# software-mansion/smelter

Measured on NVIDIA H100. Metric: 4K composited frames/sec (16-input grid) per GPU, higher is better.
Workload: dtype f32 math on u8 planes (f16 resampler scratch)

## Files before the change

smelter_b200/csrc/resample_tma3.cuh:

```cuda
#pragma once

namespace tma_int {
using namespace tma;

constexpr int kGroups = 3;

template <int S>
struct Cfg {
    static constexpr int P = 8;
    static constexpr int OUT = P / S;
    static constexpr int TAPS = 6 * S + 1;
    static constexpr int A = kLead<S>;
    static constexpr int NST = (A + S * (OUT - 1) + TAPS + P - 1) / P;
    static __host__ __device__ constexpr int last_stage(int j) { return (A + S * j + TAPS - 1) / P; }
    static __host__ __device__ constexpr int nout() {
        int m = 1 << 30;
        for (int j = 0; j < OUT; j++) {
            int c = OUT * (32 - last_stage(j)) + j;
            m = c < m ? c : m;
        }
        return m;
    }
    static constexpr int NOUT = nout();
    static constexpr int RROWS = S == 4 ? 54 : 28;
    static constexpr int RROW_BYTES = 32 * 3 * OUT * 4;
    static constexpr int RING_BYTES = RROWS * RROW_BYTES;
    static constexpr int GROUP_BYTES = kStageBytes + RING_BYTES;
    static constexpr int SMEM = kGroups * GROUP_BYTES + kTailBytes;
};

template <int S, int SRC>
__global__ void __launch_bounds__(32 * kWarps * kGroups, 1) k_resample_tma3(const FusedJob *jobs, const FusedPiece *pieces, const int *piece_begin,
                                                                            int n_virtual_blocks) {
    using K = Cfg<S>;
    using It = ChunkIter<S, 1>;
    constexpr int P = K::P, OUT = K::OUT, TAPS = K::TAPS, A = K::A, NST = K::NST;
    constexpr bool NV12 = SRC == 1;
    extern __shared__ __align__(128) unsigned char smem_all[];
    const int lane = threadIdx.x, warp = threadIdx.y % kWarps, grp = threadIdx.y / kWarps, tid = warp * 32 + lane;
    unsigned char *tail = smem_all + kGroups * K::GROUP_BYTES;
    const float *s_thr = reinterpret_cast<const float *>(tail + kThrOff);
    unsigned char *smem = smem_all + (size_t)grp * K::GROUP_BYTES;
    const uint32_t stage0 = smem_u32(smem);
    float *ring = reinterpret_cast<float *>(smem + kStageBytes);
    const uint32_t bar0 = smem_u32(tail + kBarOff) + 16u * (uint32_t)grp;
    const uint32_t kaddr = setup_block<kGroups>(tail, [] {});
    const int vb = blockIdx.x * kGroups + grp;
    if (vb >= n_virtual_blocks) return;

    Stash<It> *stash = stash_slots<It, kGroups>(tail, grp);
    uint32_t step = 0;
    It it;
    it.init(jobs, pieces, __ldg(piece_begin + vb), __ldg(piece_begin + vb + 1));

    Chunk cur = it.next();
    if (!cur.valid) return;
    if (tid == 0) issue<NV12, 1>(jobs, cur, stage0, bar0);
    uint32_t nchunk = 0;

    while (cur.valid) {
        Stash<It> *const parked = stash + (step & 1u);
        {
            const Chunk nxt = it.next();
            if (tid == 0) { parked->it = it; parked->nxt = nxt; }
        }
        const bool cur_tma = cur.nrows > 0;
        const FusedJob &J = jobs[cur.job];
        const int W = J.src.width, H = J.src.height, chei = H >> 1;
        const bool full_range = J.src.full_range != 0;
        const float nk16 = full_range ? 0.0f : -K16, rcp_y = full_range ? 1.0f : RCP_Y, rcp_c = full_range ? 1.0f : RCP_C;
        const uint32_t sb = stage0;
        if (cur_tma) {
            mbar_wait(bar0, nchunk & 1u);
            replicate_edges<NV12>(smem, cur.x0, cur.nrows, W, tid, grp);
            const LaneWords<NV12> lw(cur.x0, lane);
            for (int r = cur.r0 + warp; r < cur.r0 + cur.nrows; r += kWarps) {
                uint32_t yw[2], v[6];
                fetch_row<NV12>(sb, lw, r, cur.r0, chei, yw, v);
                float2 prg[P];
                float pb[P];
                convert_run(yw, v, nk16, rcp_y, rcp_c, kaddr, prg, pb);
                float2 arg[OUT];
                float ab[OUT];
#pragma unroll
                for (int j = 0; j < OUT; j++) { arg[j] = make_float2(0.f, 0.f); ab[j] = 0.f; }
#pragma unroll
                for (int s = 0; s < NST; s++) {
#pragma unroll
                    for (int i = 0; i < P; i++) {
#pragma unroll
                        for (int j = 0; j < OUT; j++) {
                            const int t = P * s + i - A - S * j;
                            if (t >= 0 && t < TAPS) arg[j] = fma2(prg[i], splat(c_wint[S][t]), arg[j]);
                        }
#pragma unroll
                        for (int j = 0; j < OUT; j += 2) {
                            const int t0 = P * s + i - A - S * j, t1 = t0 - S;
                            const bool a0 = t0 >= 0 && t0 < TAPS, a1 = t1 >= 0 && t1 < TAPS;
                            if (a0 && a1) {
                                const float2 d = fma2(splat(pb[i]), c_wpair[S][a0 ? t0 : 0], make_float2(ab[j], ab[j + 1]));
                                ab[j] = d.x; ab[j + 1] = d.y;
                            } else if (a0) {
                                ab[j] = fmaf(pb[i], c_wint[S][a0 ? t0 : 0], ab[j]);
                            } else if (a1) {
                                ab[j + 1] = fmaf(pb[i], c_wint[S][a1 ? t1 : 0], ab[j + 1]);
                            }
                        }
                    }
                    if (s + 1 < NST) {
#pragma unroll
                        for (int j = 0; j < OUT; j++)
                            if (K::last_stage(j) > s) {
                                arg[j].x = __shfl_up_sync(0xffffffffu, arg[j].x, 1);
                                arg[j].y = __shfl_up_sync(0xffffffffu, arg[j].y, 1);
                                ab[j] = __shfl_up_sync(0xffffffffu, ab[j], 1);
                            }
                    }
                }
                {
                    const float inv = c_winv[S];
                    float *dst = ring + (size_t)(r % K::RROWS) * (K::RROW_BYTES / 4) + lane * 3 * OUT;
#pragma unroll
                    for (int j = 0; j < OUT; j += 2) {
                        const float2 fr = __half22float2(__floats2half2_rn(arg[j].x * inv, arg[j + 1].x * inv));
                        const float2 fg = __half22float2(__floats2half2_rn(arg[j].y * inv, arg[j + 1].y * inv));
                        const float2 fb = __half22float2(__floats2half2_rn(ab[j] * inv, ab[j + 1] * inv));
                        *reinterpret_cast<float2 *>(dst + j) = fr;
                        *reinterpret_cast<float2 *>(dst + OUT + j) = fg;
                        *reinterpret_cast<float2 *>(dst + 2 * OUT + j) = fb;
                    }
                }
            }
            nchunk++;
        }
        group_sync(grp);
        if (tid == 0) issue<NV12, 1>(jobs, parked->nxt, stage0, bar0);
        if (cur.last) {
            const int tv = J.taps_v;
            const float *lbase = ring + lane * 3 * OUT;
            constexpr int ROWF = K::RROW_BYTES / 4;
            const int row_end = min(cur.o0 + kWarps, cur.oy_end);
            auto col_of = [&](int j) { return OUT * (lane - K::last_stage(j)) + j; };
            auto owned = [&](int oa, bool (&own)[OUT / 2]) {
                const int ncols = min(K::NOUT, J.dst_w - cur.ox0);
#pragma unroll
                for (int j = 0; j < OUT; j += 2) {
                    const int col = col_of(j);
                    own[j / 2] = false;
                    if (J.direct_map == nullptr || col < 0 || col >= ncols || oa >= row_end) continue;
                    const int X = J.fx + cur.ox0 + col, Y = J.fy + oa;
                    own[j / 2] = (int)__ldg(J.direct_map + (Y / kDirectTileH) * J.map_w + X / kDirectTileW) == J.direct_id;
                }
            };
            auto emit = [&](const uint32_t (&pa)[OUT], const uint32_t (&pb)[OUT], int oa, const bool (&own)[OUT / 2]) {
#pragma unroll
                for (int j = 0; j < OUT; j += 2) {
                    if (!own[j / 2]) continue;
                    emit_yuv_2x2(J, J.fx + cur.ox0 + col_of(j), J.fy + oa, pa[j], pa[j + 1], pb[j], pb[j + 1]);
                }
            };
            auto one_row = [&](int oy, uint32_t (&px)[OUT]) {
                const int fv = __ldg(J.first_v + oy);
                const float *wv = J.w_v + (size_t)oy * tv;
                float2 acc[3 * OUT / 2];
#pragma unroll
                for (int k = 0; k < 3 * OUT / 2; k++) acc[k] = make_float2(0.f, 0.f);
                for (int t = 0; t < tv; t++) {
                    const float wt = __ldg(wv + t);
                    const int row = min(max(fv + t, 0), H - 1);
                    const float *p = lbase + (row % K::RROWS) * ROWF;
#pragma unroll
                    for (int k = 0; k < 3 * OUT / 2; k++) acc[k] = fma2(*reinterpret_cast<const float2 *>(p + 2 * k), splat(wt), acc[k]);
                }
                encode_store<OUT>(J, acc, oy, s_thr, cur.ox0, K::NOUT, col_of, px);
            };
            if (J.v_same) {
                if (warp < kWarps / 2) {
                    const int oa = cur.o0 + 2 * warp, ob = oa + 1;
                    const int fa = __ldg(J.first_v) + S * oa;
                    bool own[OUT / 2];
                    owned(oa, own);
                    if (ob < row_end && fa >= 0 && fa + S + TAPS - 1 <= H - 1) {
                        float2 aa[3 * OUT / 2], bb2[3 * OUT / 2];
#pragma unroll
                        for (int k = 0; k < 3 * OUT / 2; k++) { aa[k] = make_float2(0.f, 0.f); bb2[k] = make_float2(0.f, 0.f); }
                        const int slot0 = fa % K::RROWS, nwrap = K::RROWS - slot0;
                        const float *p0 = lbase + slot0 * ROWF;
#pragma unroll
                        for (int u = 0; u < TAPS + S; u++) {
                            const float *p = p0 + (u >= nwrap ? (u - K::RROWS) * ROWF : u * ROWF);
                            float2 v[3 * OUT / 2];
#pragma unroll
                            for (int k = 0; k < 3 * OUT / 2; k++) v[k] = *reinterpret_cast<const float2 *>(p + 2 * k);
                            if (u < TAPS) {
#pragma unroll
                                for (int k = 0; k < 3 * OUT / 2; k++) aa[k] = fma2(v[k], splat(c_wint[S][u < TAPS ? u : 0]), aa[k]);
                            }
                            if (u >= S) {
#pragma unroll
                                for (int k = 0; k < 3 * OUT / 2; k++) bb2[k] = fma2(v[k], splat(c_wint[S][u >= S ? u - S : 0]), bb2[k]);
                            }
                        }
                        uint32_t pa[OUT], pb[OUT];
                        encode_store<OUT>(J, aa, oa, s_thr, cur.ox0, K::NOUT, col_of, pa);
                        encode_store<OUT>(J, bb2, ob, s_thr, cur.ox0, K::NOUT, col_of, pb);
                        emit(pa, pb, oa, own);
                    } else {
                        uint32_t pa[OUT], pb[OUT];
                        if (oa < row_end) one_row(oa, pa);
                        if (ob < row_end) { one_row(ob, pb); emit(pa, pb, oa, own); }
                    }
                }
            } else {
                const int oy = cur.o0 + warp;
                uint32_t pz[OUT];
                if (oy < row_end) one_row(oy, pz);
            }
            group_sync(grp);
        }
        cur = parked->nxt; it = parked->it; step++;
    }
}

}
```

smelter_b200/csrc/kernels.cu:

```cuda
#include <cuda_fp16.h>
#include <cuda_runtime.h>

#include <cstdio>
#include <cstdlib>
#include <atomic>
#include <cstring>

#include "kernels.h"

namespace smr {
namespace dev {

#include "ptx_helpers.cuh"

__device__ float c_u8n[256];
__device__ float c_dec[256];
__device__ float c_thr[256];
#define ENC_KEY0 ((127 - 13) << 5)
#define ENC_KEYS ((13 << 5) + 1)
__device__ unsigned char c_enc0[420];
__device__ float c_yl[256];
#define ENC1_KEY0 ((127 - 13) << 8)
#define ENC1_KEYS ((13 << 8) + 1)
__device__ unsigned char c_enc1[ENC1_KEYS + 3];
// ... 342 lines not shown
__device__ __forceinline__ float4 rs_load(const Tables &T, const Tex &s, int x, int y) {
    if (s.kind == TEX_F16) {
        const uint2 raw = __ldg(reinterpret_cast<const uint2 *>(s.p0 + (size_t)y * s.pitch0) + x);
        __half2 a = *reinterpret_cast<const __half2 *>(&raw.x), b = *reinterpret_cast<const __half2 *>(&raw.y);
        float2 fa = __half22float2(a), fb = __half22float2(b);
        return make_float4(fa.x, fa.y, fb.x, fb.y);
    }
    uchar4 p = node_texel(T, s, x, y);
    return make_float4(T.dec[p.x], T.dec[p.y], T.dec[p.z], T.u8n[p.w]);
}

__device__ __forceinline__ void rs_store(const Tables &T, const ResampleJob &J, int x, int y, float4 r) {
    if (J.dst_f16) {
        __half2 a = __floats2half2_rn(r.x, r.y), b = __floats2half2_rn(r.z, r.w);
        uint2 raw;
        raw.x = *reinterpret_cast<unsigned int *>(&a);
        raw.y = *reinterpret_cast<unsigned int *>(&b);
        reinterpret_cast<uint2 *>(J.dst + (size_t)y * J.dst_pitch)[x] = raw;
    } else {
        uchar4 o = make_uchar4((unsigned char)srgb_encode(T, r.x), (unsigned char)srgb_encode(T, r.y),
                               (unsigned char)srgb_encode(T, r.z), (unsigned char)unorm8(r.w));
        reinterpret_cast<uchar4 *>(J.dst + (size_t)y * J.dst_pitch)[x] = o;
    }
}

__global__ void __launch_bounds__(256) k_resample(const ResampleJob *jobs) {
    __shared__ Tables T;
    load_tables(T);
    const ResampleJob &J = jobs[blockIdx.z];
    int px = blockIdx.x * blockDim.x + threadIdx.x, py = blockIdx.y * blockDim.y + threadIdx.y;
    if (px >= J.dst_w || py >= J.dst_h) return;
    const Tex &S = J.src;
    if (J.box_fx * J.box_fy > 1) {
        float4 sum = make_float4(0.f, 0.f, 0.f, 0.f);
        for (int dy = 0; dy < J.box_fy; dy++)
            for (int dx = 0; dx < J.box_fx; dx++) {
                int sx = min(px * J.box_fx + dx, S.width - 1), sy = min(py * J.box_fy + dy, S.height - 1);
                float4 t = rs_load(T, S, sx, sy);
                sum.x += t.x; sum.y += t.y; sum.z += t.z; sum.w += t.w;
            }
        float d = (float)((unsigned)J.box_fx * (unsigned)J.box_fy);
        rs_store(T, J, px, py, make_float4(sum.x / d, sum.y / d, sum.z / d, sum.w / d));
        return;
    }
    int o = J.axis == 1 ? py : px;
    int max_src = (J.axis == 1 ? S.height : S.width) - 1;
    int max_perp = (J.axis == 1 ? S.width : S.height) - 1;
    int perp = min(max((J.axis == 1 ? px : py) + J.perp_offset, 0), max_perp);
    const float *w = J.weights + (size_t)o * J.taps;
    int first = __ldg(J.first + o);
    float4 sum = make_float4(0.f, 0.f, 0.f, 0.f);
    for (int t = 0; t < J.taps; t++) {
        float wt = __ldg(w + t);
        if (wt == 0.0f) continue;
        int src = min(max(first + t, 0), max_src);
        float4 tx = J.axis == 1 ? rs_load(T, S, perp, src) : rs_load(T, S, src, perp);
        sum.x = fmaf(tx.x, wt, sum.x);
        sum.y = fmaf(tx.y, wt, sum.y);
        sum.z = fmaf(tx.z, wt, sum.z);
        sum.w = fmaf(tx.w, wt, sum.w);
    }
    float inv = __ldg(J.inv_wsum + o);
    rs_store(T, J, px, py, make_float4(sum.x * inv, sum.y * inv, sum.z * inv, sum.w * inv));
}

int launch_resample(const ResampleJob *jobs_dev, const ResampleJob *jobs_host, int n, Stream s) {
    if (n <= 0) return 0;
    int mw = 1, mh = 1;
    for (int i = 0; i < n; i++) {
        mw = jobs_host[i].dst_w > mw ? jobs_host[i].dst_w : mw;
        mh = jobs_host[i].dst_h > mh ? jobs_host[i].dst_h : mh;
    }
    dim3 b(32, 8), g((mw + 31) / 32, (mh + 7) / 8, n);
    k_resample<<<g, b, 0, (cudaStream_t)s>>>(jobs_dev);
    return check_launch("k_resample") ? 1 : -1;
}

#define W64_TW 64
#define W64_WARPS 8
#define W64_RING 64

__constant__ float c_wint[5][32];
__constant__ float c_winv[5];
__constant__ float2 c_wpair[5][32];

void set_int_weights(int S, const float *weights_dev, const float *inv_dev, int taps, Stream s) {
    cudaMemcpyToSymbolAsync(c_wint, weights_dev, sizeof(float) * taps, sizeof(float) * 32 * S, cudaMemcpyDeviceToDevice, (cudaStream_t)s);
    cudaMemcpyToSymbolAsync(c_winv, inv_dev, sizeof(float), sizeof(float) * S, cudaMemcpyDeviceToDevice, (cudaStream_t)s);
    float *pair = nullptr;
    cudaGetSymbolAddress((void **)&pair, c_wpair);
    pair += 2 * 32 * S;
    cudaMemsetAsync(pair, 0, sizeof(float2) * 32, (cudaStream_t)s);
    cudaMemcpy2DAsync(pair, sizeof(float2), weights_dev, sizeof(float), sizeof(float), taps, cudaMemcpyDeviceToDevice, (cudaStream_t)s);
    if (taps > S)
        cudaMemcpy2DAsync(pair + 2 * S + 1, sizeof(float2), weights_dev, sizeof(float), sizeof(float), taps - S,
                          cudaMemcpyDeviceToDevice, (cudaStream_t)s);
}

template <int S>
struct W64 {
    static constexpr int SS = S == 0 ? 4 : S;
    static constexpr int TAPS = 6 * SS + 1;
    static constexpr int SPAN = (W64_TW - 1) * SS + TAPS + 3;
    static constexpr int ROWLEN = S == 0 ? ((SPAN + 2 + 7) & ~7) : (((SPAN + SPAN / (2 * SS) + 2) + 7) & ~7);
    struct Smem {
        Tables T;
        __half2 ring[W64_RING][3][W64_TW / 2];
        float4 srow[W64_WARPS][ROWLEN];
        float hw[S == 0 ? TAPS * W64_TW : 1];
    };
    static __device__ __forceinline__ int pos(int i) { return S == 0 ? i : i + i / (2 * SS); }
};

__device__ __forceinline__ void prefetch_l2_span(const uint8_t *p, int bytes, const uint8_t *lo, const uint8_t *hi) {
    unsigned long long a = (unsigned long long)(p < lo ? lo : p), e = (unsigned long long)(p + bytes < hi ? p + bytes : hi);
    a = (a + 15ull) & ~15ull;
    if (e <= a + 16ull) return;
    const unsigned size = (unsigned)((e - a) & ~15ull);
    asm volatile("cp.async.bulk.prefetch.L2.global [%0], %1;" ::"l"(a), "r"(size) : "memory");
}

template <int S, int SRC>
__global__ void __launch_bounds__(32 * W64_WARPS, 3) k_resample_fused_int(const FusedJob *jobs, const FusedPiece *pieces,
                                                                            const int *piece_begin) {
    constexpr bool NV12 = SRC == 1, IL = SRC >= 2;
    using K = W64<S>;
    constexpr int TAPS = K::TAPS;
    constexpr int WIN = S + TAPS;
    extern __shared__ __align__(16) unsigned char fs_raw[];
    typename K::Smem &M = *reinterpret_cast<typename K::Smem *>(fs_raw);
    load_tables(M.T);
    const int lane = threadIdx.x, warp = threadIdx.y;
    for (int pi = __ldg(piece_begin + blockIdx.x); pi < __ldg(piece_begin + blockIdx.x + 1); pi++) {
    const FusedPiece P = pieces[pi];
    const FusedJob &J = jobs[P.job];
    const int th = S == 0 ? J.taps_h : TAPS;
    const int ox0 = P.strip * W64_TW;
    const int oy_begin = P.oy_begin, oy_end = P.oy_end;
    const Tex &src = J.src;
    const int W = src.width, H = src.height, chei = H >> 1;
    const int tv = J.taps_v;
    const int xa = __ldg(J.first_h + ox0);
    const int xa_e = xa & ~1;
    const int d0 = xa - xa_e;
    const int oc0 = min(ox0 + 2 * lane, J.dst_w - 1), oc1 = min(ox0 + 2 * lane + 1, J.dst_w - 1);
    int gi0 = 0, gD = 0, npairs_g = 0;
    float inv0, inv1;
    if constexpr (S == 0) {
        const int f0 = __ldg(J.first_h + oc0), f1 = __ldg(J.first_h + oc1);
        gi0 = f0 - xa_e; gD = f1 - f0;
        inv0 = __ldg(J.inv_h + oc0); inv1 = __ldg(J.inv_h + oc1);
        const int o_last = min(ox0 + W64_TW - 1, J.dst_w - 1);
        npairs_g = (min(__ldg(J.first_h + o_last) + th - xa_e, K::SPAN) + 1) >> 1;
        for (int t = warp; t < th; t += W64_WARPS) {
            M.hw[t * W64_TW + 2 * lane] = __ldg(J.w_h + (size_t)oc0 * th + t);
            M.hw[t * W64_TW + 2 * lane + 1] = __ldg(J.w_h + (size_t)oc1 * th + t);
        }
        __syncthreads();
    } else {
        inv0 = inv1 = c_winv[S];
    }
    constexpr int NP = ((W64_TW - 1) * K::SS + TAPS + 2) >> 1, NIT = (NP + 31) / 32;
    const int npairs = S == 0 ? npairs_g : NP;
    const int full_range = src.full_range;
    const float *ytab = full_range ? M.T.u8n : M.T.yl;
    const int p_in_lo = IL ? (xa_e >= 0 ? 0 : (1 - xa_e) >> 1) : (xa_e >= 2 ? 0 : (2 - xa_e + 1) >> 1);
    const int p_in_hi = IL ? (W - 2 - xa_e) >> 1 : (W - 4 - xa_e) >> 1;
    const int p_hi = min(p_in_hi, npairs - 1);
    const int dsh = S == 0 ? 0 : d0;

    int produced_hi = -0x40000000;
    for (int o0 = oy_begin; o0 < oy_end; o0 += W64_WARPS) {
        const int o_l = min(o0 + W64_WARPS - 1, oy_end - 1);
        const int need_lo = min(max(__ldg(J.first_v + o0), 0), H - 1);
        const int need_hi = min(max(__ldg(J.first_v + o_l) + tv - 1, 0), H - 1);
        const int start = max(produced_hi + 1, need_lo);
        {
            const int tid = warp * 32 + lane;
            const int nr = need_hi + 1 + (tid >> 2), part = tid & 3;
// ... 226 lines not shown
    return fmaf(v + 0.5f, 0.87843137254f, K16);
}

__device__ __forceinline__ void emit_yuv_2x2(const FusedJob &J, int X, int Y, uint32_t p00, uint32_t p10, uint32_t p01, uint32_t p11) {
    using namespace tma;
    const float2 m23 = splat(-8388608.0f);
    const float2 c = splat(__uint_as_float(0x3b808081u)), lo = splat(__uint_as_float(0xaf7efeffu));
    auto pairf = [&](uint32_t a, uint32_t b, uint32_t sel) {
        return add2(make_float2(__uint_as_float(__byte_perm(a, 0x4B000000u, sel)), __uint_as_float(__byte_perm(b, 0x4B000000u, sel))), m23);
    };
    auto unit = [&](float2 n) { return fma2(n, c, mul2(n, lo)); };
    auto store2 = [&](float2 x01) -> uint32_t {
        const float2 q = add2_after_mul(mul2(x01, splat(255.0f)), splat(12582912.0f));
        return (__float_as_uint(q.x) & 0xffu) | ((__float_as_uint(q.y) & 0xffu) << 8);
    };
    auto lum2 = [&](uint32_t a, uint32_t b) -> uint32_t {
        const float2 r = unit(pairf(a, b, 0x7540u)), g = unit(pairf(a, b, 0x7541u)), bl = unit(pairf(a, b, 0x7542u));
        const float2 y = fma2(bl, splat(0.0722f), fma2(g, splat(0.7152f), mul2(r, splat(0.2126f))));
        return store2(make_float2(__saturatef(fmaf(y.x, 0.85882352941f, K16)), __saturatef(fmaf(y.y, 0.85882352941f, K16))));
    };
    *reinterpret_cast<unsigned short *>(J.out0 + (size_t)Y * J.out_pitch0 + X) = (unsigned short)lum2(p00, p10);
    *reinterpret_cast<unsigned short *>(J.out0 + (size_t)(Y + 1) * J.out_pitch0 + X) = (unsigned short)lum2(p01, p11);
    const uint32_t m = 0x00ff00ffu;
    const uint32_t srb = (p00 & m) + (p10 & m) + (p01 & m) + (p11 & m);
    const uint32_t sga = ((p00 >> 8) & m) + ((p10 >> 8) & m) + ((p01 >> 8) & m) + ((p11 >> 8) & m);
    const float2 c4 = splat(__uint_as_float(0x3b808081u) * 0.25f), lo4 = splat(__uint_as_float(0xaf7efeffu) * 0.25f);
    const float2 nrg = add2(make_float2(__uint_as_float(__byte_perm(srb, 0x4B000000u, 0x7610u)), __uint_as_float(__byte_perm(sga, 0x4B000000u, 0x7610u))), m23);
    const float nb = __uint_as_float(__byte_perm(srb, 0x4B000000u, 0x7632u)) - 8388608.0f;
    const float2 rg = fma2(nrg, c4, mul2(nrg, lo4));
    const float b = fmaf(nb, c4.x, nb * lo4.x);
    float2 uv = mul2(splat(rg.x), make_float2(-0.1146f, 0.5f));
    uv = fma2(splat(rg.y), make_float2(-0.3854f, -0.4542f), uv);
    uv = fma2(splat(b), make_float2(0.5f, -0.0458f), uv);
    uv = add2(uv, splat(0.5f));
    const uint32_t cuv = store2(make_float2(__saturatef(fmaf(uv.x, 0.87843137254f, K16)), __saturatef(fmaf(uv.y, 0.87843137254f, K16))));
    if (J.out_format == 4) {
        *reinterpret_cast<unsigned short *>(J.out1 + (size_t)(Y >> 1) * J.out_pitch1 + X) = (unsigned short)cuv;
    } else {
        J.out1[(size_t)(Y >> 1) * J.out_pitch1 + (X >> 1)] = (unsigned char)(cuv & 0xffu);
        J.out2[(size_t)(Y >> 1) * J.out_pitch2 + (X >> 1)] = (unsigned char)(cuv >> 8);
    }
}

#include "resample_tma.cuh"
#include "resample_tma3.cuh"
#include "resample_tma0.cuh"

template <int SRC, int WINP, int BOX>
static bool launch_tma0(const FusedJob *jobs_dev, const FusedPiece *pieces, const int *piece_begin, int nblocks, cudaStream_t s) {
    static std::atomic<unsigned long long> done{0};
    int dev = 0;
    cudaGetDevice(&dev);
    const unsigned long long bit = 1ull << (dev & 63);
    if (!(done.load(std::memory_order_acquire) & bit)) {
        cudaFuncSetAttribute(tma_any::k_resample_tma0<SRC, WINP, BOX>, cudaFuncAttributeMaxDynamicSharedMemorySize, tma_any::Cfg::SMEM);
        done.fetch_or(bit, std::memory_order_release);
    }
    const int grid = (nblocks + tma_any::kGroups - 1) / tma_any::kGroups;
    tma_any::k_resample_tma0<SRC, WINP, BOX><<<grid, dim3(32, tma::kWarps * tma_any::kGroups), tma_any::Cfg::SMEM, s>>>(jobs_dev, pieces, piece_begin, nblocks);
    return check_launch("k_resample_tma0");
}

template <int S, int SRC>
static bool launch_tma3(const FusedJob *jobs_dev, const FusedPiece *pieces, const int *piece_begin, int nblocks, cudaStream_t s) {
    static std::atomic<unsigned long long> done{0};
    int dev = 0;
    cudaGetDevice(&dev);
    const unsigned long long bit = 1ull << (dev & 63);
    if (!(done.load(std::memory_order_acquire) & bit)) {
        cudaFuncSetAttribute(tma_int::k_resample_tma3<S, SRC>, cudaFuncAttributeMaxDynamicSharedMemorySize, tma_int::Cfg<S>::SMEM);
        done.fetch_or(bit, std::memory_order_release);
    }
    const int grid = (nblocks + tma_int::kGroups - 1) / tma_int::kGroups;
    tma_int::k_resample_tma3<S, SRC><<<grid, dim3(32, tma::kWarps * tma_int::kGroups), tma_int::Cfg<S>::SMEM, s>>>(jobs_dev, pieces, piece_begin, nblocks);
    return check_launch("k_resample_tma3");
}

int launch_resample_fused(int variant, int src, const FusedJob *jobs_dev, const FusedPiece *pieces_dev,
                          const int *piece_begin_dev, int nblocks, Stream s) {
    if (nblocks <= 0) return 0;
    cudaStream_t st = (cudaStream_t)s;
    bool ok = false;
    static_assert(tma_int::Cfg<4>::NOUT == kTmaStripCols4 && tma_int::Cfg<2>::NOUT == kTmaStripCols2 &&
                  tma_int::Cfg<4>::RROWS == kTmaRing4 && tma_int::Cfg<2>::RROWS == kTmaRing2, "integer-ratio kernel");
    static_assert(tma_any::kGroups == kTma0Groups && tma_any::Cfg::MAXT == kTma0MaxTaps && tma_any::Cfg::WINP_MAX == kTma0Window[3] &&
                  tma_any::Cfg::RROWS == kTmaRing4, "any-ratio kernel");
    static_assert(tma::kLumaBox == 2 * kTmaLumaBoxW && tma::kChunkRows == kTmaLumaBoxH && tma::kNv12Box == 2 * kTmaNv12BoxW &&
                  tma::kPlanarBox == kTmaPlanarBoxW && tma::kChromaRows == kTmaChromaBoxH, "TMA boxes");
    switch (variant) {
#define SMR_TMA0_CASE(B) \
        case 30 + B: ok = src == 1 ? launch_tma0<1, kTma0Window[B], 0>(jobs_dev, pieces_dev, piece_begin_dev, nblocks, st) \
                                   : launch_tma0<0, kTma0Window[B], 0>(jobs_dev, pieces_dev, piece_begin_dev, nblocks, st); break; \
        case 40 + B: ok = src == 1 ? launch_tma0<1, kTma0Window[B], 1>(jobs_dev, pieces_dev, piece_begin_dev, nblocks, st) \
                                   : launch_tma0<0, kTma0Window[B], 1>(jobs_dev, pieces_dev, piece_begin_dev, nblocks, st); break;
        SMR_TMA0_CASE(0) SMR_TMA0_CASE(1) SMR_TMA0_CASE(2) SMR_TMA0_CASE(3)
#undef SMR_TMA0_CASE
        case 22: ok = src == 1 ? launch_tma3<2, 1>(jobs_dev, pieces_dev, piece_begin_dev, nblocks, st)
                               : launch_tma3<2, 0>(jobs_dev, pieces_dev, piece_begin_dev, nblocks, st); break;
        case 24: ok = src == 1 ? launch_tma3<4, 1>(jobs_dev, pieces_dev, piece_begin_dev, nblocks, st)
                               : launch_tma3<4, 0>(jobs_dev, pieces_dev, piece_begin_dev, nblocks, st); break;
        case 2: ok = launch_fused_src<2>(src, jobs_dev, pieces_dev, piece_begin_dev, nblocks, st); break;
        case 3: ok = launch_fused_src<3>(src, jobs_dev, pieces_dev, piece_begin_dev, nblocks, st); break;
        case 4: ok = launch_fused_src<4>(src, jobs_dev, pieces_dev, piece_begin_dev, nblocks, st); break;
        default: ok = launch_fused_src<0>(src, jobs_dev, pieces_dev, piece_begin_dev, nblocks, st); break;
    }
    return ok ? 1 : -1;
}

__device__ __forceinline__ void half_row_convert(const uint32_t (&yw)[2], const uint32_t (&v)[6], float nk16, float rcp_y, float rcp_c,
                                                 int (&sums)[4][3]) {
#pragma unroll
    for (int p = 0; p < 4; p++) {
        float2 qr, qg, qb;
        tma::convert_pair(yw, v, p, nk16, rcp_y, rcp_c, qr, qg, qb);
        sums[p][0] += (int)(__float_as_uint(qr.x) & 0xffu) + (int)(__float_as_uint(qr.y) & 0xffu);
        sums[p][1] += (int)(__float_as_uint(qg.x) & 0xffu) + (int)(__float_as_uint(qg.y) & 0xffu);
        sums[p][2] += (int)(__float_as_uint(qb.x) & 0xffu) + (int)(__float_as_uint(qb.y) & 0xffu);
    }
}

template <bool NV12>
__device__ __forceinline__ void half_row_sums(const Tex &S, int x0, int r, float nk16, float rcp_y, float rcp_c, int (&sums)[4][3]) {
    const uint8_t *yrow = S.p0 + (size_t)r * S.pitch0 + x0;
    const uint32_t yw[2] = {__ldg(reinterpret_cast<const uint32_t *>(yrow)), __ldg(reinterpret_cast<const uint32_t *>(yrow) + 1)};
    const int ch = r >> 1, cl = (r & 1) ? ch + 1 : ch - 1, cx = x0 >> 1;
    uint32_t v[6];
#pragma unroll
    for (int k = 0; k < 6; k++) {
        uint32_t h, l;
        if (NV12) {
            const uint32_t th = __ldg(reinterpret_cast<const unsigned short *>(S.p1 + (size_t)ch * S.pitch1) + (cx - 1 + k));
            const uint32_t tl = __ldg(reinterpret_cast<const unsigned short *>(S.p1 + (size_t)cl * S.pitch1) + (cx - 1 + k));
            h = __byte_perm(th, 0, 0x4140); l = __byte_perm(tl, 0, 0x4140);
        } else {
            h = __ldg(S.p1 + (size_t)ch * S.pitch1 + cx - 1 + k) | ((uint32_t)__ldg(S.p2 + (size_t)ch * S.pitch2 + cx - 1 + k) << 16);
            l = __ldg(S.p1 + (size_t)cl * S.pitch1 + cx - 1 + k) | ((uint32_t)__ldg(S.p2 + (size_t)cl * S.pitch2 + cx - 1 + k) << 16);
        }
        v[k] = 3u * h + l;
    }
    half_row_convert(yw, v, nk16, rcp_y, rcp_c, sums);
}

__device__ __forceinline__ void half_pair_sums_nv12(const Tex &S, int x0, int r, float nk16, float rcp_y, float rcp_c, int (&sums)[4][3]) {
    const int ch = r >> 1;
    auto spread_row = [&](int crow, uint32_t (&t)[6]) {
        const uint32_t *w = reinterpret_cast<const uint32_t *>(S.p1 + (size_t)crow * S.pitch1 + x0 - 4);
        const uint32_t w0 = __ldg(w), w1 = __ldg(w + 1), w2 = __ldg(w + 2), w3 = __ldg(w + 3);
        t[0] = __byte_perm(w0, 0, 0x4342); t[1] = __byte_perm(w1, 0, 0x4140); t[2] = __byte_perm(w1, 0, 0x4342);
        t[3] = __byte_perm(w2, 0, 0x4140); t[4] = __byte_perm(w2, 0, 0x4342); t[5] = __byte_perm(w3, 0, 0x4140);
    };
    uint32_t th[6], tl[6], v[6];
    spread_row(ch, th);
#pragma unroll
    for (int k = 0; k < 6; k++) th[k] *= 3u;
#pragma unroll
    for (int half = 0; half < 2; half++) {
        spread_row(half ? ch + 1 : ch - 1, tl);
#pragma unroll
        for (int k = 0; k < 6; k++) v[k] = th[k] + tl[k];
        const uint32_t *yrow = reinterpret_cast<const uint32_t *>(S.p0 + (size_t)(r + half) * S.pitch0 + x0);
        const uint32_t yw[2] = {__ldg(yrow), __ldg(yrow + 1)};
        half_row_convert(yw, v, nk16, rcp_y, rcp_c, sums);
    }
}

__device__ __forceinline__ float smoothstep_f(float e0, float e1, float x) {
    float t = clamp01((x - e0) / (e1 - e0));
// ... 842 lines not shown
```

smelter_b200/csrc/kernels.h:

```cpp
#pragma once

#include <cstddef>
#include <cstdint>

namespace smr {
namespace dev {

enum TexKind : int32_t {
    TEX_NONE = 0,
    TEX_RGBA8 = 1,
    TEX_YUV420 = 2,
    TEX_NV12 = 3,
    TEX_F16 = 4,
    TEX_BGRA = 5,
    TEX_ARGB = 6,
    TEX_YUV422 = 7,
    TEX_YUV444 = 8,
    TEX_UYVY = 9,
    TEX_YUYV = 10,
};
inline
#ifdef __CUDACC__
__host__ __device__
#endif
// ... 19 lines not shown
    int32_t type;
    int32_t rotated;
    float left, top, width, height;
    float content_w, content_h;
    float cx, cy, cs, sn;
    int32_t px0, px1, py0, py1;
    long long vx[4], vy[4];
    float border_radius[4];
    float color[4];
    float border_color[4];
    float border_width, blur_radius;
    int32_t tex;
    float crop_sx, crop_ox, crop_sy, crop_oy;
    int32_t mask_begin, mask_count;
    int32_t ix0, ix1, iy0, iy1;
    int32_t jx0, jx1, jy0, jy1;
    int32_t fast;
    int32_t tx_off, ty_off;
    uint32_t const_bytes;
};
enum : int32_t { FAST_IDENT = 1, FAST_CONST = 2, FAST_LUT = 4, FAST_OPAQUE = 8, FAST_SAMPLE = 16, FAST_HALF = 32 };

struct CompositeJob {
    int32_t width, height;
    int32_t mode;
    int32_t n_layers;
    const LayerDev *layers;
    const LayerDev *layers_host;
    const MaskDev *masks;
    const Tex *textures;
    int32_t out_format;
    uint8_t *out0, *out1, *out2;
    int32_t out_pitch0, out_pitch1, out_pitch2;
    const uint8_t *direct_map;
    int32_t map_w;
    const uint32_t *tile_list;
    int32_t n_tiles;
};
constexpr int kDirectTileW = 128, kDirectTileH = 16;

struct ResampleJob {
    Tex src;
    int32_t axis;
    int32_t perp_offset;
    int32_t taps;
    int32_t dst_w, dst_h;
    int32_t dst_f16;
    uint8_t *dst;
    int32_t dst_pitch;
    const float *weights;
    const float *inv_wsum;
    const int32_t *first;
    int32_t box_fx, box_fy;
};

struct FusedJob {
    Tex src;
    int32_t dst_w, dst_h;
    uint8_t *dst;
    int32_t dst_pitch;
    int32_t taps_h, taps_v;
    const float *w_h, *inv_h;
    const int32_t *first_h;
    const float *w_v, *inv_v;
    const int32_t *first_v;
    int32_t variant;
    const void *tm0, *tm1, *tm2;
    int32_t v_same;
    int32_t strip_cols;
    const uint8_t *lane_perm;
    const uint8_t *direct_map;
    int32_t direct_id;
    int32_t map_w;
    int32_t fx, fy;
    int32_t out_format;
    uint8_t *out0, *out1, *out2;
    int32_t out_pitch0, out_pitch1, out_pitch2;
};
struct FusedPiece {
    int32_t job, strip, oy_begin, oy_end;
};
constexpr int kFusedStripCols = 64, kFusedWarps = 8, kFusedRing = 64, kFusedSpan = 280, kFusedMaxTaps = 25;
constexpr int kTmaStripCols4 = 58, kTmaStripCols2 = 122, kTmaRing4 = 54, kTmaRing2 = 28;
constexpr int kTmaLumaBoxW = 136, kTmaLumaBoxH = 32, kTmaNv12BoxW = 144, kTmaPlanarBoxW = 160, kTmaChromaBoxH = 18;
constexpr int kTma0Groups = 2, kTma0MaxSpan = 256, kTma0MaxTaps = 25;
constexpr int kTma0Window[4] = {20, 25, 29, 33};
inline int fused_strip_cols(int variant) { return variant == 24 ? kTmaStripCols4 : variant == 22 ? kTmaStripCols2 : kFusedStripCols; }

struct WeightJob {
    float scale, offset;
    int32_t n_out, taps;
    float *weights;
    float *inv_wsum;
    int32_t *first;
};

struct OutputJob {
    Tex src;
    int32_t out_w, out_h;
    int32_t out_format;
    uint8_t *out0, *out1, *out2;
    int32_t out_pitch0, out_pitch1, out_pitch2;
};

struct GlyphDev {
    int32_t x, y;
    uint16_t w, h, ax, ay;
    uint8_t color[4];
    int32_t content;
};
struct TextJob {
    int32_t width, height;
    int32_t mode;
    int32_t color_mode;
    int32_t n_glyphs;
    float bg[4];
    const GlyphDev *glyphs;
    const uint8_t *mask; int32_t mask_w, mask_h, mask_pitch;
    const uint8_t *color; int32_t color_w, color_h, color_pitch;
    uint8_t *out; int32_t out_pitch;
};

void upload_tables(const float *u8n, const float *srgb_dec, const float *srgb_enc_thr);

typedef void *Stream;

int launch_convert_to_rgba(const Tex &src, uint8_t *dst, int dst_pitch, Stream s);
int launch_weights(const WeightJob *jobs_dev, const WeightJob *jobs_host, int n_jobs, Stream s);
int launch_resample(const ResampleJob *jobs_dev, const ResampleJob *jobs_host, int n_jobs, Stream s);
inline int fused_source_class(int tex_kind) {
    return tex_kind == TEX_YUV420 ? 0 : tex_kind == TEX_NV12 ? 1 : tex_kind == TEX_UYVY ? 2 : tex_kind == TEX_YUYV ? 3 : -1;
}
int launch_preprocess(const Tex &src, int mode, int rescale, uint8_t *out, int out_pitch, int out_w, int out_h, Stream s);
int launch_text(const TextJob &job, Stream s);
int launch_resample_fused(int variant, int src, const FusedJob *jobs_dev, const FusedPiece *pieces_dev,
                          const int *piece_begin_dev, int nblocks, Stream s);
void set_int_weights(int S, const float *weights_dev, const float *inv_dev, int taps, Stream s);
int launch_composite(const CompositeJob &job, Stream s);
int launch_composite_multi(const CompositeJob *jobs_dev, const CompositeJob *jobs_host, int n, Stream s);
int launch_output(const OutputJob &job, Stream s);
int launch_fill_yuv(uint8_t *p0, uint8_t *p1, uint8_t *p2, int pitch0, int pitch1, int pitch2, int w, int h,
                    int out_format, uint8_t y, uint8_t u, uint8_t v, Stream s);
const char *last_launch_error();

}
}
```

smelter_b200/csrc/ptx_helpers.cuh:

```cuda
#pragma once

namespace tma {

__device__ __forceinline__ uint32_t smem_u32(const void *p) { return (uint32_t)__cvta_generic_to_shared(p); }

__device__ __forceinline__ void mbar_init(uint32_t bar, uint32_t count) {
    asm volatile("mbarrier.init.shared::cta.b64 [%0], %1;" ::"r"(bar), "r"(count) : "memory");
}
__device__ __forceinline__ void mbar_expect_tx(uint32_t bar, uint32_t bytes) {
    asm volatile("mbarrier.arrive.expect_tx.shared::cta.b64 _, [%0], %1;" ::"r"(bar), "r"(bytes) : "memory");
}
__device__ __forceinline__ void mbar_wait(uint32_t bar, uint32_t parity) {
    asm volatile(
        "{\n"
        ".reg .pred p;\n"
        "WAIT_%=:\n"
        "mbarrier.try_wait.parity.shared::cta.b64 p, [%0], %1;\n"
        "@p bra DONE_%=;\n"
        "bra WAIT_%=;\n"
        "DONE_%=:\n"
        "}\n" ::"r"(bar), "r"(parity)
        : "memory");
}
__device__ __forceinline__ void tma_load_2d(uint32_t dst, const void *tmap, int x, int y, uint32_t bar) {
    asm volatile("cp.async.bulk.tensor.2d.shared::cluster.global.mbarrier::complete_tx::bytes [%0], [%1, {%2, %3}], [%4];" ::"r"(dst),
                 "l"(tmap), "r"(x), "r"(y), "r"(bar)
                 : "memory");
}
__device__ __forceinline__ void fence_proxy_async() { asm volatile("fence.proxy.async.shared::cta;" ::: "memory"); }

__device__ __forceinline__ void lds64v(uint32_t a, uint32_t &x, uint32_t &y) {
    asm volatile("ld.shared.v2.u32 {%0, %1}, [%2];" : "=r"(x), "=r"(y) : "r"(a) : "memory");
}
__device__ __forceinline__ uint32_t lds32v(uint32_t a) {
    uint32_t x;
    asm volatile("ld.shared.u32 %0, [%1];" : "=r"(x) : "r"(a) : "memory");
    return x;
}
__device__ __forceinline__ uint32_t lds16v(uint32_t a) {
    uint32_t x;
    asm volatile("ld.shared.u16 %0, [%1];" : "=r"(x) : "r"(a) : "memory");
    return x;
}
__device__ __forceinline__ uint32_t lds8v(uint32_t a) {
    uint32_t x;
    asm volatile("ld.shared.u8 %0, [%1];" : "=r"(x) : "r"(a) : "memory");
    return x;
}
__device__ __forceinline__ float lds_tab(uint32_t a) {
    float x;
    asm("ld.shared.f32 %0, [%1];" : "=f"(x) : "r"(a));
    return x;
}

__device__ __forceinline__ unsigned long long pk(float2 a) {
    unsigned long long r;
    asm("mov.b64 %0, {%1, %2};" : "=l"(r) : "f"(a.x), "f"(a.y));
    return r;
}
__device__ __forceinline__ float2 upk(unsigned long long r) {
    float2 a;
    asm("mov.b64 {%0, %1}, %2;" : "=f"(a.x), "=f"(a.y) : "l"(r));
    return a;
}
__device__ __forceinline__ float2 fma2(float2 a, float2 b, float2 c) {
    return make_float2(__fmaf_rn(a.x, b.x, c.x), __fmaf_rn(a.y, b.y, c.y));
}
__device__ __forceinline__ float2 mul2(float2 a, float2 b) { return make_float2(__fmul_rn(a.x, b.x), __fmul_rn(a.y, b.y)); }
__device__ __forceinline__ float2 add2(float2 a, float2 b) { return make_float2(__fadd_rn(a.x, b.x), __fadd_rn(a.y, b.y)); }
__device__ __forceinline__ float2 splat(float a) { return make_float2(a, a); }
__device__ __forceinline__ unsigned long long fma2q(unsigned long long a, unsigned long long b, unsigned long long c) {
    return pk(fma2(upk(a), upk(b), upk(c)));
}
__device__ __forceinline__ void lds128q(uint32_t addr, unsigned long long &lo, unsigned long long &hi) {
    asm volatile("ld.shared.v2.b64 {%0, %1}, [%2];" : "=l"(lo), "=l"(hi) : "r"(addr));
}
__device__ __forceinline__ float2 add2_after_mul(float2 a, float2 c) { return add2(a, c); }


}
```

Baseline: 1523.

## Split S=2 vertical pass across all warps with half-column work per lane

For the 2x downscale case, the vertical filtering in the v_same path now runs on all warps rather than half. Each pair of warps splits the output columns: a lane covers half of its OUT outputs, and the lane pair exchanges pixels by shuffle for the 2x2 YUV emit. This targets the idle half of the warps and lowers per-thread register pressure. In exchange it adds an inline encoder, shuffles, and duplicated ownership logic, and the fallback path still runs on only half the warps.

```diff
diff --git a/smelter_b200/csrc/resample_tma3.cuh b/smelter_b200/csrc/resample_tma3.cuh
--- a/smelter_b200/csrc/resample_tma3.cuh
+++ b/smelter_b200/csrc/resample_tma3.cuh
@@ -175,40 +175,119 @@
                 encode_store<OUT>(J, acc, oy, s_thr, cur.ox0, K::NOUT, col_of, px);
             };
             if (J.v_same) {
-                if (warp < kWarps / 2) {
-                    const int oa = cur.o0 + 2 * warp, ob = oa + 1;
+                if constexpr (S == 2) {
+                    constexpr int HC = OUT / 2;
+                    const int pr = warp % (kWarps / 2), hf = warp / (kWarps / 2);
+                    const int oa = cur.o0 + 2 * pr, ob = oa + 1;
                     const int fa = __ldg(J.first_v) + S * oa;
-                    bool own[OUT / 2];
-                    owned(oa, own);
                     if (ob < row_end && fa >= 0 && fa + S + TAPS - 1 <= H - 1) {
-                        float2 aa[3 * OUT / 2], bb2[3 * OUT / 2];
-#pragma unroll
-                        for (int k = 0; k < 3 * OUT / 2; k++) { aa[k] = make_float2(0.f, 0.f); bb2[k] = make_float2(0.f, 0.f); }
+                        const int slot = 16 * hf + (lane >> 1), jo = (lane & 1) * HC;
+                        const int col0 = OUT * (slot - K::last_stage(jo)) + jo;
+                        const int ncols = min(K::NOUT, J.dst_w - cur.ox0);
+                        bool own = false;
+                        if (J.direct_map != nullptr && (HC == 2 || jo == 0) && col0 >= 0 && col0 < ncols) {
+                            const int X = J.fx + cur.ox0 + col0, Y = J.fy + oa;
+                            own = (int)__ldg(J.direct_map + (Y / kDirectTileH) * J.map_w + X / kDirectTileW) == J.direct_id;
+                        }
+                        float aa[3][HC], bb[3][HC];
+#pragma unroll
+                        for (int c = 0; c < 3; c++)
+#pragma unroll
+                            for (int i = 0; i < HC; i++) { aa[c][i] = 0.f; bb[c][i] = 0.f; }
                         const int slot0 = fa % K::RROWS, nwrap = K::RROWS - slot0;
-                        const float *p0 = lbase + slot0 * ROWF;
+                        const float *p0 = ring + slot * 3 * OUT + jo + slot0 * ROWF;
 #pragma unroll
                         for (int u = 0; u < TAPS + S; u++) {
                             const float *p = p0 + (u >= nwrap ? (u - K::RROWS) * ROWF : u * ROWF);
-                            float2 v[3 * OUT / 2];
-#pragma unroll
-                            for (int k = 0; k < 3 * OUT / 2; k++) v[k] = *reinterpret_cast<const float2 *>(p + 2 * k);
+                            float v[3][HC];
+#pragma unroll
+                            for (int c = 0; c < 3; c++) {
+                                if (HC == 2) {
+                                    const float2 t = *reinterpret_cast<const float2 *>(p + c * OUT);
+                                    v[c][0] = t.x; v[c][HC - 1] = t.y;
+                                } else {
+                                    v[c][0] = p[c * OUT];
+                                }
+                            }
                             if (u < TAPS) {
 #pragma unroll
-                                for (int k = 0; k < 3 * OUT / 2; k++) aa[k] = fma2(v[k], splat(c_wint[S][u < TAPS ? u : 0]), aa[k]);
+                                for (int c = 0; c < 3; c++)
+#pragma unroll
+                                    for (int i = 0; i < HC; i++) aa[c][i] = __fmaf_rn(v[c][i], c_wint[S][u < TAPS ? u : 0], aa[c][i]);
                             }
                             if (u >= S) {
 #pragma unroll
-                                for (int k = 0; k < 3 * OUT / 2; k++) bb2[k] = fma2(v[k], splat(c_wint[S][u >= S ? u - S : 0]), bb2[k]);
-                            }
-                        }
-                        uint32_t pa[OUT], pb[OUT];
-                        encode_store<OUT>(J, aa, oa, s_thr, cur.ox0, K::NOUT, col_of, pa);
-                        encode_store<OUT>(J, bb2, ob, s_thr, cur.ox0, K::NOUT, col_of, pb);
-                        emit(pa, pb, oa, own);
-                    } else {
+                                for (int c = 0; c < 3; c++)
+#pragma unroll
+                                    for (int i = 0; i < HC; i++) bb[c][i] = __fmaf_rn(v[c][i], c_wint[S][u >= S ? u - S : 0], bb[c][i]);
+                            }
+                        }
+                        auto encode = [&](const float (&acc)[3][HC], int oy, uint32_t (&px)[HC]) {
+                            const float inv_v = __ldg(J.inv_v + oy);
+                            auto enc = [&](float lin) -> uint32_t {
+                                const float x = clamp01(lin);
+                                const int k = max((__float_as_int(x) >> 15) - ENC1_KEY0, 0);
+                                const uint32_t e = __ldg(c_enc1 + k);
+                                return e + (x >= s_thr[e] ? 1u : 0u);
+                            };
+                            uint32_t *drow = reinterpret_cast<uint32_t *>(J.dst + (size_t)oy * J.dst_pitch) + cur.ox0;
+#pragma unroll
+                            for (int i = 0; i < HC; i++) {
+                                px[i] = enc(acc[0][i] * inv_v) | (enc(acc[1][i] * inv_v) << 8) | (enc(acc[2][i] * inv_v) << 16) | 0xff000000u;
+                                if (col0 + i >= 0 && col0 + i < ncols) drow[col0 + i] = px[i];
+                            }
+                        };
+                        uint32_t pa[HC], pb[HC];
+                        encode(aa, oa, pa);
+                        encode(bb, ob, pb);
+                        if (J.direct_map != nullptr) {
+                            const uint32_t pa1 = HC == 2 ? pa[HC - 1] : __shfl_xor_sync(0xffffffffu, pa[0], 1);
+                            const uint32_t pb1 = HC == 2 ? pb[HC - 1] : __shfl_xor_sync(0xffffffffu, pb[0], 1);
+                            if (own) emit_yuv_2x2(J, J.fx + cur.ox0 + col0, J.fy + oa, pa[0], pa1, pb[0], pb1);
+                        }
+                    } else if (hf == 0) {
+                        bool own[OUT / 2];
+                        owned(oa, own);
                         uint32_t pa[OUT], pb[OUT];
                         if (oa < row_end) one_row(oa, pa);
                         if (ob < row_end) { one_row(ob, pb); emit(pa, pb, oa, own); }
+                    }
+                } else {
+                    if (warp < kWarps / 2) {
+                        const int oa = cur.o0 + 2 * warp, ob = oa + 1;
+                        const int fa = __ldg(J.first_v) + S * oa;
+                        bool own[OUT / 2];
+                        owned(oa, own);
+                        if (ob < row_end && fa >= 0 && fa + S + TAPS - 1 <= H - 1) {
+                            float2 aa[3 * OUT / 2], bb2[3 * OUT / 2];
+#pragma unroll
+                            for (int k = 0; k < 3 * OUT / 2; k++) { aa[k] = make_float2(0.f, 0.f); bb2[k] = make_float2(0.f, 0.f); }
+                            const int slot0 = fa % K::RROWS, nwrap = K::RROWS - slot0;
+                            const float *p0 = lbase + slot0 * ROWF;
+#pragma unroll
+                            for (int u = 0; u < TAPS + S; u++) {
+                                const float *p = p0 + (u >= nwrap ? (u - K::RROWS) * ROWF : u * ROWF);
+                                float2 v[3 * OUT / 2];
+#pragma unroll
+                                for (int k = 0; k < 3 * OUT / 2; k++) v[k] = *reinterpret_cast<const float2 *>(p + 2 * k);
+                                if (u < TAPS) {
+#pragma unroll
+                                    for (int k = 0; k < 3 * OUT / 2; k++) aa[k] = fma2(v[k], splat(c_wint[S][u < TAPS ? u : 0]), aa[k]);
+                                }
+                                if (u >= S) {
+#pragma unroll
+                                    for (int k = 0; k < 3 * OUT / 2; k++) bb2[k] = fma2(v[k], splat(c_wint[S][u >= S ? u - S : 0]), bb2[k]);
+                                }
+                            }
+                            uint32_t pa[OUT], pb[OUT];
+                            encode_store<OUT>(J, aa, oa, s_thr, cur.ox0, K::NOUT, col_of, pa);
+                            encode_store<OUT>(J, bb2, ob, s_thr, cur.ox0, K::NOUT, col_of, pb);
+                            emit(pa, pb, oa, own);
+                        } else {
+                            uint32_t pa[OUT], pb[OUT];
+                            if (oa < row_end) one_row(oa, pa);
+                            if (ob < row_end) { one_row(ob, pb); emit(pa, pb, oa, own); }
+                        }
                     }
                 }
             } else {
```

Measured after the change: 1517, median of 6. About the same (-0.4%).

## Trim dead taps, use power-of-two ring and vector smem loads in tma3 resampler

Applied to the files above, without the earlier changes.

Limits the integer-ratio filter loops to the TAPS-1 live weights, on the assumption that the last weight is zero, and drops the paired-weight constant table. The S=4 ring grows to 64 rows so the slot index becomes a mask instead of a modulo. The v_same vertical path now reads shared memory through 128-bit or 64-bit vector loads on precomputed addresses. Cutting the last tap changes results if the final weight is not actually zero, and the larger ring uses more shared memory per group, which can lower occupancy.

```diff
diff --git a/smelter_b200/csrc/kernels.cu b/smelter_b200/csrc/kernels.cu
--- a/smelter_b200/csrc/kernels.cu
+++ b/smelter_b200/csrc/kernels.cu
@@ -448,19 +448,10 @@
 
 __constant__ float c_wint[5][32];
 __constant__ float c_winv[5];
-__constant__ float2 c_wpair[5][32];
 
 void set_int_weights(int S, const float *weights_dev, const float *inv_dev, int taps, Stream s) {
     cudaMemcpyToSymbolAsync(c_wint, weights_dev, sizeof(float) * taps, sizeof(float) * 32 * S, cudaMemcpyDeviceToDevice, (cudaStream_t)s);
     cudaMemcpyToSymbolAsync(c_winv, inv_dev, sizeof(float), sizeof(float) * S, cudaMemcpyDeviceToDevice, (cudaStream_t)s);
-    float *pair = nullptr;
-    cudaGetSymbolAddress((void **)&pair, c_wpair);
-    pair += 2 * 32 * S;
-    cudaMemsetAsync(pair, 0, sizeof(float2) * 32, (cudaStream_t)s);
-    cudaMemcpy2DAsync(pair, sizeof(float2), weights_dev, sizeof(float), sizeof(float), taps, cudaMemcpyDeviceToDevice, (cudaStream_t)s);
-    if (taps > S)
-        cudaMemcpy2DAsync(pair + 2 * S + 1, sizeof(float2), weights_dev, sizeof(float), sizeof(float), taps - S,
-                          cudaMemcpyDeviceToDevice, (cudaStream_t)s);
 }
 
 template <int S>
@@ -853,7 +844,8 @@
     cudaStream_t st = (cudaStream_t)s;
     bool ok = false;
     static_assert(tma_int::Cfg<4>::NOUT == kTmaStripCols4 && tma_int::Cfg<2>::NOUT == kTmaStripCols2 &&
-                  tma_int::Cfg<4>::RROWS == kTmaRing4 && tma_int::Cfg<2>::RROWS == kTmaRing2, "integer-ratio kernel");
+                  tma_int::Cfg<4>::RROWS == kTma3Ring4 && kTma3Ring4 >= kTmaRing4 && tma_int::Cfg<2>::RROWS == kTmaRing2,
+                  "integer-ratio kernel");
     static_assert(tma_any::kGroups == kTma0Groups && tma_any::Cfg::MAXT == kTma0MaxTaps && tma_any::Cfg::WINP_MAX == kTma0Window[3] &&
                   tma_any::Cfg::RROWS == kTmaRing4, "any-ratio kernel");
     static_assert(tma::kLumaBox == 2 * kTmaLumaBoxW && tma::kChunkRows == kTmaLumaBoxH && tma::kNv12Box == 2 * kTmaNv12BoxW &&
diff --git a/smelter_b200/csrc/kernels.h b/smelter_b200/csrc/kernels.h
--- a/smelter_b200/csrc/kernels.h
+++ b/smelter_b200/csrc/kernels.h
@@ -125,6 +125,7 @@
 };
 constexpr int kFusedStripCols = 64, kFusedWarps = 8, kFusedRing = 64, kFusedSpan = 280, kFusedMaxTaps = 25;
 constexpr int kTmaStripCols4 = 58, kTmaStripCols2 = 122, kTmaRing4 = 54, kTmaRing2 = 28;
+constexpr int kTma3Ring4 = 64;
 constexpr int kTmaLumaBoxW = 136, kTmaLumaBoxH = 32, kTmaNv12BoxW = 144, kTmaPlanarBoxW = 160, kTmaChromaBoxH = 18;
 constexpr int kTma0Groups = 2, kTma0MaxSpan = 256, kTma0MaxTaps = 25;
 constexpr int kTma0Window[4] = {20, 25, 29, 33};
diff --git a/smelter_b200/csrc/ptx_helpers.cuh b/smelter_b200/csrc/ptx_helpers.cuh
--- a/smelter_b200/csrc/ptx_helpers.cuh
+++ b/smelter_b200/csrc/ptx_helpers.cuh
@@ -31,6 +31,9 @@
 
 __device__ __forceinline__ void lds64v(uint32_t a, uint32_t &x, uint32_t &y) {
     asm volatile("ld.shared.v2.u32 {%0, %1}, [%2];" : "=r"(x), "=r"(y) : "r"(a) : "memory");
+}
+__device__ __forceinline__ void lds128v(uint32_t a, uint32_t &x, uint32_t &y, uint32_t &z, uint32_t &w) {
+    asm volatile("ld.shared.v4.u32 {%0, %1, %2, %3}, [%4];" : "=r"(x), "=r"(y), "=r"(z), "=r"(w) : "r"(a) : "memory");
 }
 __device__ __forceinline__ uint32_t lds32v(uint32_t a) {
     uint32_t x;
diff --git a/smelter_b200/csrc/resample_tma3.cuh b/smelter_b200/csrc/resample_tma3.cuh
--- a/smelter_b200/csrc/resample_tma3.cuh
+++ b/smelter_b200/csrc/resample_tma3.cuh
@@ -10,6 +10,7 @@
     static constexpr int P = 8;
     static constexpr int OUT = P / S;
     static constexpr int TAPS = 6 * S + 1;
+    static constexpr int LIVE = TAPS - 1;
     static constexpr int A = kLead<S>;
     static constexpr int NST = (A + S * (OUT - 1) + TAPS + P - 1) / P;
     static __host__ __device__ constexpr int last_stage(int j) { return (A + S * j + TAPS - 1) / P; }
@@ -22,7 +23,8 @@
         return m;
     }
     static constexpr int NOUT = nout();
-    static constexpr int RROWS = S == 4 ? 54 : 28;
+    static constexpr int RROWS = S == 4 ? kTma3Ring4 : kTmaRing2;
+    static __device__ __forceinline__ int slot(int r) { return (RROWS & (RROWS - 1)) == 0 ? (r & (RROWS - 1)) : r % RROWS; }
     static constexpr int RROW_BYTES = 32 * 3 * OUT * 4;
     static constexpr int RING_BYTES = RROWS * RROW_BYTES;
     static constexpr int GROUP_BYTES = kStageBytes + RING_BYTES;
@@ -91,19 +93,9 @@
 #pragma unroll
                         for (int j = 0; j < OUT; j++) {
                             const int t = P * s + i - A - S * j;
-                            if (t >= 0 && t < TAPS) arg[j] = fma2(prg[i], splat(c_wint[S][t]), arg[j]);
-                        }
-#pragma unroll
-                        for (int j = 0; j < OUT; j += 2) {
-                            const int t0 = P * s + i - A - S * j, t1 = t0 - S;
-                            const bool a0 = t0 >= 0 && t0 < TAPS, a1 = t1 >= 0 && t1 < TAPS;
-                            if (a0 && a1) {
-                                const float2 d = fma2(splat(pb[i]), c_wpair[S][a0 ? t0 : 0], make_float2(ab[j], ab[j + 1]));
-                                ab[j] = d.x; ab[j + 1] = d.y;
-                            } else if (a0) {
-                                ab[j] = fmaf(pb[i], c_wint[S][a0 ? t0 : 0], ab[j]);
-                            } else if (a1) {
-                                ab[j + 1] = fmaf(pb[i], c_wint[S][a1 ? t1 : 0], ab[j + 1]);
+                            if (t >= 0 && t < K::LIVE) {
+                                arg[j] = fma2(prg[i], splat(c_wint[S][t]), arg[j]);
+                                ab[j] = fmaf(pb[i], c_wint[S][t], ab[j]);
                             }
                         }
                     }
@@ -119,7 +111,7 @@
                 }
                 {
                     const float inv = c_winv[S];
-                    float *dst = ring + (size_t)(r % K::RROWS) * (K::RROW_BYTES / 4) + lane * 3 * OUT;
+                    float *dst = ring + (size_t)K::slot(r) * (K::RROW_BYTES / 4) + lane * 3 * OUT;
 #pragma unroll
                     for (int j = 0; j < OUT; j += 2) {
                         const float2 fr = __half22float2(__floats2half2_rn(arg[j].x * inv, arg[j + 1].x * inv));
@@ -168,13 +160,14 @@
                 for (int t = 0; t < tv; t++) {
                     const float wt = __ldg(wv + t);
                     const int row = min(max(fv + t, 0), H - 1);
-                    const float *p = lbase + (row % K::RROWS) * ROWF;
+                    const float *p = lbase + K::slot(row) * ROWF;
 #pragma unroll
                     for (int k = 0; k < 3 * OUT / 2; k++) acc[k] = fma2(*reinterpret_cast<const float2 *>(p + 2 * k), splat(wt), acc[k]);
                 }
                 encode_store<OUT>(J, acc, oy, s_thr, cur.ox0, K::NOUT, col_of, px);
             };
             if (J.v_same) {
+                static_assert(K::LIVE + S <= K::RROWS, "v_same window wraps at most once");
                 if (warp < kWarps / 2) {
                     const int oa = cur.o0 + 2 * warp, ob = oa + 1;
                     const int fa = __ldg(J.first_v) + S * oa;
@@ -184,17 +177,25 @@
                         float2 aa[3 * OUT / 2], bb2[3 * OUT / 2];
 #pragma unroll
                         for (int k = 0; k < 3 * OUT / 2; k++) { aa[k] = make_float2(0.f, 0.f); bb2[k] = make_float2(0.f, 0.f); }
-                        const int slot0 = fa % K::RROWS, nwrap = K::RROWS - slot0;
-                        const float *p0 = lbase + slot0 * ROWF;
-#pragma unroll
-                        for (int u = 0; u < TAPS + S; u++) {
-                            const float *p = p0 + (u >= nwrap ? (u - K::RROWS) * ROWF : u * ROWF);
+                        const int slot0 = K::slot(fa), nwrap = K::RROWS - slot0;
+                        const uint32_t q0 = smem_u32(lbase + slot0 * ROWF), q1 = q0 - (uint32_t)K::RING_BYTES;
+#pragma unroll
+                        for (int u = 0; u < K::LIVE + S; u++) {
+                            const uint32_t q = (u < nwrap ? q0 : q1) + (uint32_t)(u * K::RROW_BYTES);
                             float2 v[3 * OUT / 2];
-#pragma unroll
-                            for (int k = 0; k < 3 * OUT / 2; k++) v[k] = *reinterpret_cast<const float2 *>(p + 2 * k);
-                            if (u < TAPS) {
-#pragma unroll
-                                for (int k = 0; k < 3 * OUT / 2; k++) aa[k] = fma2(v[k], splat(c_wint[S][u < TAPS ? u : 0]), aa[k]);
+                            uint32_t w[3 * OUT];
+                            if constexpr (3 * OUT % 4 == 0) {
+#pragma unroll
+                                for (int k = 0; k < 3 * OUT; k += 4) lds128v(q + 4u * k, w[k], w[k + 1], w[k + 2], w[k + 3]);
+                            } else {
+#pragma unroll
+                                for (int k = 0; k < 3 * OUT; k += 2) lds64v(q + 4u * k, w[k], w[k + 1]);
+                            }
+#pragma unroll
+                            for (int k = 0; k < 3 * OUT / 2; k++) v[k] = make_float2(__uint_as_float(w[2 * k]), __uint_as_float(w[2 * k + 1]));
+                            if (u < K::LIVE) {
+#pragma unroll
+                                for (int k = 0; k < 3 * OUT / 2; k++) aa[k] = fma2(v[k], splat(c_wint[S][u < K::LIVE ? u : 0]), aa[k]);
                             }
                             if (u >= S) {
 #pragma unroll
```

Measured after the change: 1711 before, 1755 after (median of 6 runs). 2.6% higher.
